# feihoo87/waveforms

Hardware: AMD Instinct MI355X
Metric: Msamples/s (all channels) (higher is better)
Workload: dtype f64; 1 GPU; sampler256: 256 ch/GPU x 1e+07 pts, 100 gaussian+DRAG pulses/ch, seeds 1000+c (SURVEY 8(d) C4/C5 channel spec), grid mode; channels_per_gpu=256, channels_total=256, points_per_channel=10000000, output=device (HBM) buffer, parallelism=channel-block-per-rank x1, no data-path collective

## Files before the change

### waveforms_amd/csrc/wfk_kernels.hip

```cpp
#include <hip/hip_runtime.h>

#include <string>
#include <type_traits>
#include <utility>

#include "wfk.h"
#include "wfk_internal.h"
#include "wfk_pick.h"

namespace {

__device__ __forceinline__ int uni(int v) { return __builtin_amdgcn_readfirstlane(v); }
__device__ __forceinline__ int64_t uni64(int64_t v) {
  const uint32_t lo = __builtin_amdgcn_readfirstlane((uint32_t)v);
  const uint32_t hi = __builtin_amdgcn_readfirstlane((uint32_t)((uint64_t)v >> 32));
  return (int64_t)(((uint64_t)hi << 32) | lo);
}
#define WFK_CONST __attribute__((address_space(4)))
template <typename V>
__device__ __forceinline__ V cload(const void* base, int byte_off) {
  return *reinterpret_cast<const WFK_CONST V*>(reinterpret_cast<uintptr_t>(base) + byte_off);
}
__device__ __forceinline__ DevPiece load_piece(const DevPiece* p) {
  DevPiece P;
// ... 392 lines not shown
      constexpr int IB = NS % 8 == 0 ? 8 : 1;
#pragma unroll
      for (int k0 = 0; k0 < NS; k0 += IB) {
        double dd[IB], f0[IB], s0[IB];
#pragma unroll
        for (int kk = 0; kk < IB; ++kk) {
          const double x = fma((double)(k0 + kk), D, u0);
          const double xc = fmin(fmax(x, start), stop);
          int j = (int)((xc - start) * inv_step);
          j = j > last ? last : j;
          const double d0 = xc - fma((double)j, step, start);
          dd[kk] = x != x ? x : d0;
          f0[kk] = fp[j];
          s0[kk] = sl[j];
        }
        __builtin_amdgcn_sched_barrier(0);
#pragma unroll
        for (int kk = 0; kk < IB; ++kk) prod[k0 + kk] *= (T)fma(s0[kk], dd[kk], f0[kk]);
      }
    } else if (mode == WFK_M_INTERP_GRID) {
#pragma clang fp contract(off)
      const double start = r[3], stop = r[4], inv_step = r[8], step = r[9];
      const int m = (int)r[5];
      const double* fp = a.pool + (int64_t)r[6];
      const double* sl = a.pool + (int64_t)r[7];
#pragma unroll
      for (int k0 = 0; k0 < NS; k0 += 4) {
        double xs[4], xj[4], f0[4], sv[4];
        int js[4];
        bool flat[4];
#pragma unroll
        for (int kk = 0; kk < 4; ++kk) {
          if (k0 + kk < NS) {
            double x = grid_time<SLICE>(a, j0 + 64 * (int64_t)(k0 + kk));
            if (tshift != 0.0) x = x - tshift;
            x = x - shift;
            int j;
            bool fl = true;
            if (!(x <= stop)) j = m - 1;
            else if (x < start) j = 0;
            else {
              j = (int)((x - start) * inv_step);
              j = j < 0 ? 0 : (j > m - 1 ? m - 1 : j);
              while (j > 0 && x < np_linspace_at_s(start, stop, m, j, step)) --j;
              while (j < m - 1 && x >= np_linspace_at_s(start, stop, m, j + 1, step)) ++j;
              fl = j == m - 1;
            }
            xs[kk] = x; js[kk] = j;
            xj[kk] = np_linspace_at_s(start, stop, m, j, step);
            flat[kk] = fl || xj[kk] == x;
          }
        }
#pragma unroll
        for (int kk = 0; kk < 4; ++kk)
          if (k0 + kk < NS) { f0[kk] = fp[js[kk]]; sv[kk] = sl[js[kk]]; }
#pragma unroll
        for (int kk = 0; kk < 4; ++kk) {
          if (k0 + kk < NS) {
            double v = flat[kk] ? f0[kk] : sv[kk] * (xs[kk] - xj[kk]) + f0[kk];
            if (isnan(xs[kk])) v = xs[kk];
            else if (isnan(v))
              v = prim_interp_fast(xs[kk], start, stop, fp, sl, m, inv_step, step);
            prod[k0 + kk] *= (T)v;
          }
        }
      }
    } else {
      const double D = r[3];
#pragma unroll
      for (int k = 0; k < NS; ++k) prod[k] *= (T)(u0 + (double)k * D);
    }
    return;
  }
  if (!DIRECT) return;
  const double pw = r[1];
  const bool has_pw = pw != 1.0;
  double* mine = s_val + threadIdx.x;
  if (mode == WFK_M_SAMPLED) {
    const double* tab = a.pool + (int64_t)r[3];
    const int64_t i0 = (int64_t)r[4], m = (int64_t)r[5];
#pragma unroll 1
    for (int k = 0; k < NS; ++k) {
      int64_t i = j0 + 64 * (int64_t)k - i0;
      i = i < 0 ? 0 : (i >= m ? m - 1 : i);
      double v = m > 0 ? tab[i] : __builtin_nan("");
      if (has_pw) v = np_power(v, pw);
      mine[k * WFK_WG] = v;
    }
  } else {
#pragma unroll 1
    for (int k = 0; k < NS; ++k) {
      double x = time_at<TLIST, SLICE>(a, j0 + 64 * (int64_t)k);
      if (tshift != 0.0) x = x - tshift;
      double v = prim_direct(mode, x - shift, r, a.pool);
      if (has_pw) v = np_power(v, pw);
      mine[k * WFK_WG] = v;
    }
  }
#pragma unroll
  for (int k = 0; k < NS; ++k) prod[k] *= (T)mine[k * WFK_WG];
}

struct FceSeeds { double c, s, g, r; };

__device__ __attribute__((noinline)) FceSeeds fce_seeds(double theta, double theta_lo, double ea,
                                                        double eb, int carrier, int env) {
#pragma clang fp contract(off)
  FceSeeds o;
  o.c = 1.0; o.s = 0.0; o.g = 1.0; o.r = 1.0;
  if (carrier == 1) {
    const double IPI_HI = 0.31830988618379069, IPI_LO = -1.9678676675182486e-17;
    const double xh = theta * IPI_HI;
    const double xl = fma(theta, IPI_HI, -xh) + fma(theta, IPI_LO, theta_lo * IPI_HI);
    const double n = rint(xh);
    double ss, cc;
    sincospi((xh - n) + xl, &ss, &cc);
    const bool odd = ((long long)n) & 1;
    o.s = odd ? -ss : ss;
    o.c = odd ? -cc : cc;
  }
  if (carrier == 2) o.c = erf(theta);
  if (env) {
    o.g = exp(ea);
    o.r = exp(eb);
  }
  return o;
}

struct CorrCtx {
  double dj0;
  double xref;
  double step, t0, tshift, last, dlast;
  int kbase;
};

template <int K>
__device__ __forceinline__ double corr_delta(const CorrCtx& cc, double dj0, double D, double W,
                                             double wm, double sm) {
#pragma clang fp contract(off)
  const double dj = dj0 + (double)(64 * K);
  const double m = dj * cc.step;
  double t = m + cc.t0;
  if (dj == cc.dlast) t = cc.last;
  t = t - cc.tshift;
  const double eps = (t - cc.xref) - (double)(cc.kbase + K) * D;
  const double um = t - sm;
  const double bb = um - t;
  const double eu = (t - (um - bb)) + (-sm - bb);
  const double pm = wm * um;
  const double rho = -__builtin_fma(wm, um, -pm);
  return __builtin_fma(W, eps, __builtin_fma(-wm, eu, rho));
}

template <typename T, int NS, int DEG, bool CARRIER, int ENV, bool CORR = false>
__device__ __forceinline__ void fce_loop(const double2* tab, const double* r, FceSeeds& sd,
                                         double u0, T (&acc)[NS],
                                         const CorrCtx* cc = nullptr) {
  using S = typename std::conditional<ENV == 2, double, T>::type;
  constexpr int SB = 4;
  asm volatile("" : "+v"(u0) : : "memory");
  double dj0 = 0.0, wm = 0.0, sm = 0.0;
  if constexpr (CORR) {
    wm = r[WFK_FCE_WM];
    sm = r[WFK_FCE_SM];
    dj0 = cc->dj0;
    asm volatile("" : "+v"(dj0));
  }
  const T c0 = (T)sd.c, s0 = (T)sd.s;
  const T A0 = (T)r[WFK_FCE_A], A1 = (T)r[WFK_FCE_A + 1], B0 = (T)r[WFK_FCE_B],
          B1 = (T)r[WFK_FCE_B + 1];
  const T A2 = DEG > 1 ? (T)r[WFK_FCE_A + 2] : (T)0, A3 = DEG > 1 ? (T)r[WFK_FCE_A + 3] : (T)0;
  const T B2 = DEG > 1 ? (T)r[WFK_FCE_B + 2] : (T)0, B3 = DEG > 1 ? (T)r[WFK_FCE_B + 3] : (T)0;
  const T ac = A0 * c0, as = A0 * s0;
  const bool fold = CARRIER && !CORR && DEG > 0;
  const T P0 = fold ? A0 * c0 + B0 * s0 : (T)0, P1 = fold ? A1 * c0 + B1 * s0 : (T)0;
  const T Q0 = fold ? B0 * c0 - A0 * s0 : (T)0, Q1 = fold ? B1 * c0 - A1 * s0 : (T)0;
  const T P2 = fold && DEG > 1 ? A2 * c0 + B2 * s0 : (T)0, P3 = fold && DEG > 1 ? A3 * c0 + B3 * s0 : (T)0;
  const T Q2 = fold && DEG > 1 ? B2 * c0 - A2 * s0 : (T)0, Q3 = fold && DEG > 1 ? B3 * c0 - A3 * s0 : (T)0;
  const double D = r[WFK_FCE_D];
  S g = (S)sd.g, rr = (S)sd.r;
  const S q = (S)r[WFK_FCE_Q];
  T u = (T)u0;
  const T Dt = (T)D;
  double2 tb[2][SB];
  if (CARRIER) {
    WFK_EACH(SB, kk) tb[0][kk] = tab[kk]; WFK_END
  }
  WFK_EACH(NS / SB, kb)
    if constexpr (CARRIER && (kb + 1) * SB < NS) {
      WFK_EACH(SB, kk) tb[(kb + 1) & 1][kk] = tab[(kb + 1) * SB + kk]; WFK_END
    }
    WFK_EACH(SB, kk)
      constexpr int k = kb * SB + kk;
      T val;
      if constexpr (DEG == 0 && CARRIER && !CORR && ENV == 0) {
        const double2 cs = tb[kb & 1][kk];
        acc[k] = __builtin_fma(ac, (T)cs.x, acc[k]);
        acc[k] = __builtin_fma(-as, (T)cs.y, acc[k]);
        return;
      }
      if (DEG == 0) {
        if (CARRIER) {
          const double2 cs = tb[kb & 1][kk];
          if constexpr (CORR) {
            const T we = (T)corr_delta<k>(*cc, dj0, D, r[WFK_FCE_W], wm, sm);
            const T ck = c0 * (T)cs.x - s0 * (T)cs.y;
            const T sk = s0 * (T)cs.x + c0 * (T)cs.y;
            val = A0 * (ck - we * sk);
          } else {
            val = ac * (T)cs.x - as * (T)cs.y;
          }
        } else {
          val = A0;
        }
      } else if constexpr (CARRIER && !CORR) {
        const double2 cs = tb[kb & 1][kk];
        T pp, qq;
        if (DEG == 1) {
          pp = P1 * u + P0;
          qq = Q1 * u + Q0;
        } else {
          pp = ((P3 * u + P2) * u + P1) * u + P0;
          qq = ((Q3 * u + Q2) * u + Q1) * u + Q0;
        }
        u += Dt;
        val = pp * (T)cs.x + qq * (T)cs.y;
      } else {
        T pa, pb;
        if (DEG == 1) {
          pa = A1 * u + A0;
          pb = B1 * u + B0;
        } else {
          pa = ((A3 * u + A2) * u + A1) * u + A0;
          pb = ((B3 * u + B2) * u + B1) * u + B0;
        }
        u += Dt;
        if (CARRIER) {
          const double2 cs = tb[kb & 1][kk];
          T ck = c0 * (T)cs.x - s0 * (T)cs.y;
          T sk = s0 * (T)cs.x + c0 * (T)cs.y;
          if constexpr (CORR) {
            const T we = (T)corr_delta<k>(*cc, dj0, D, r[WFK_FCE_W], wm, sm);
            const T c1 = ck - we * sk;
            sk = sk + we * ck;
            ck = c1;
          }
          val = pa * ck + pb * sk;
        } else {
          val = pa;
        }
      }
      if (ENV) {
        acc[k] += val * (T)g;
        g *= rr;
        rr *= q;
      } else {
        acc[k] += val;
      }
    WFK_END
    __builtin_amdgcn_sched_barrier(0);
  WFK_END
  if (ENV) {
    sd.g = (double)g;
    sd.r = (double)rr;
  }
  if (CARRIER) {
    const double2 e = tab[NS];
    const double c = sd.c, sn = sd.s;
    sd.c = c * e.x - sn * e.y;
    sd.s = sn * e.x + c * e.y;
  }
}

template <typename T, int NS, int DEG, bool CARRIER, bool CORR = false>
__device__ __forceinline__ void fce_env(const double2* tab, const double* r, FceSeeds& sd,
                                        double u0, int env, T (&acc)[NS], const CorrCtx* cc = nullptr) {
  if (env == 0) fce_loop<T, NS, DEG, CARRIER, 0, CORR>(tab, r, sd, u0, acc, cc);
  else if (sizeof(T) == 8 || env == 1) fce_loop<T, NS, DEG, CARRIER, 1, CORR>(tab, r, sd, u0, acc, cc);
  else fce_loop<T, NS, DEG, CARRIER, 2>(tab, r, sd, u0, acc);
}

template <bool EXACT = false>
__device__ __forceinline__ FceSeeds fce_make_seeds(const double* r, double x, int fl) {
  double v = (x - r[WFK_FCE_SG]) / r[WFK_FCE_SIGMA];
  const double Hh = r[WFK_FCE_H];
  if ((fl & 0x33) == 0x31) {
    const double vm = v + 0.5 * Hh;
    return fce_seeds(v, 0.0, -(vm * vm), -Hh * (2.0 * vm + Hh), 2, 1);
  }
  if (fl & WFK_FCE_EXPENV) v = 0.0;
  const double sref = r[WFK_FCE_SREF], W = r[WFK_FCE_W];
  const double d = x - sref;
  const double th = W * d;
  double lo = 0.0;
  if (EXACT) {
    const double bb = d - x;
    const double ed = (x - (d - bb)) + (-sref - bb);
    lo = fma(W, ed, fma(W, d, -th));
  }
  if (fl & WFK_FCE_EXPENV)
    return fce_seeds(th, lo, r[WFK_FCE_SIGMA] * (x - r[WFK_FCE_SG]), Hh, (fl >> 2) & 1, (fl >> 4) & 3);
  return fce_seeds(th, lo, -(v * v), -Hh * (2.0 * v + Hh), (fl >> 2) & 1, (fl >> 4) & 3);
}

template <typename T, int NS, bool CORR = false>
__device__ __forceinline__ void fce_eval(const double* blk, const double* r, FceSeeds& sd,
                                         double x, bool wide_env, T (&acc)[NS], int fl,
                                         const CorrCtx* cc = nullptr) {
  const int deg = fl & 3;
  const int carrier = (fl >> 2) & 1;
  int env = (fl >> 4) & 3;
  if (env && sizeof(T) == 4 && (wide_env || ((fl >> 6) & 1) == 0)) env = 2;
  const double2* tab = reinterpret_cast<const double2*>(blk + WFK_FCE_TABOFF(fl));
  const double u0 = x - r[WFK_FCE_SLIN];
  if constexpr (CORR && sizeof(T) == 8) {
    if (carrier && ((fl >> 7) & 1)) {
      if (deg == 0) fce_env<T, NS, 0, true, true>(tab, r, sd, u0, env, acc, cc);
      else if (deg == 1) fce_env<T, NS, 1, true, true>(tab, r, sd, u0, env, acc, cc);
      else fce_env<T, NS, 3, true, true>(tab, r, sd, u0, env, acc, cc);
      return;
    }
  }
  if (carrier) {
    if (deg == 0) fce_env<T, NS, 0, true>(tab, r, sd, u0, env, acc);
    else if (deg == 1) fce_env<T, NS, 1, true>(tab, r, sd, u0, env, acc);
    else fce_env<T, NS, 3, true>(tab, r, sd, u0, env, acc);
  } else {
    if (deg == 0) fce_env<T, NS, 0, false>(tab, r, sd, u0, env, acc);
    else fce_env<T, NS, 3, false>(tab, r, sd, u0, env, acc);
  }
}

template <typename T, int NS, bool CPLX>
__device__ __forceinline__ void fce_envmul(const double* r, FceSeeds& sd, T (&acc)[NS],
                                           T (&acci)[CPLX ? NS : 1]) {
  double g = sd.g, rr = sd.r;
  const double q = r[WFK_FCE_Q];
  WFK_EACH(NS, k)
    acc[k] *= (T)g;
    if constexpr (CPLX) acci[k] *= (T)g;
    g *= rr;
    rr *= q;
  WFK_END
  sd.g = g;
  sd.r = rr;
}

template <typename T, int NS, bool CPLX>
__device__ __forceinline__ void fce_erfmul(const double* r, FceSeeds& sd, double x, T (&acc)[NS],
                                           T (&acci)[CPLX ? NS : 1]) {
  double E = sd.c, g = sd.g, rr = sd.r;
  const double q = r[WFK_FCE_Q], h = r[WFK_FCE_H];
  const double m0 = r[WFK_FCE_A], m1 = r[WFK_FCE_A + 1];
  const double p0 = r[WFK_FCE_B], p1 = r[WFK_FCE_B + 1], p2 = r[WFK_FCE_B + 2], p3 = r[WFK_FCE_B + 3];
  double vm = (x - r[WFK_FCE_SG]) / r[WFK_FCE_SIGMA] + 0.5 * h;
  WFK_EACH(NS, k)
    const T m = (T)fma(m1, E, m0);
    acc[k] *= m;
    if constexpr (CPLX) acci[k] *= m;
    const double w = vm * vm;
    E = fma(g, fma(fma(fma(p3, w, p2), w, p1), w, p0), E);
    g *= rr;
    rr *= q;
    vm += h;
  WFK_END
  sd.c = E;
  sd.g = g;
  sd.r = rr;
}

template <typename T, int NS>
__device__ __forceinline__ void fce_bank(const double* blk, const double* gblk, const double* rec0, int n, double* s_st, int lane,
                                         T (&acc)[NS]) {
  constexpr int SB = 4;
#pragma unroll 1
  for (int i = 0; i < n; ++i) {
    const double* r = rec0 + i * WFK_FCE_REC;
    const int fl = uni(WFK_FCE_WORD(r));
#ifndef WFK_BANK_LDS
    const WFK_CONST double* tabd = reinterpret_cast<const WFK_CONST double*>(reinterpret_cast<uintptr_t>(gblk + WFK_FCE_TABOFF(fl)));
#else
    const double* tabd = blk + WFK_FCE_TABOFF(fl);
#endif
    auto tab = [&](int k) __attribute__((always_inline)) { return make_double2(tabd[2 * k], tabd[2 * k + 1]); };
    double* const st = s_st + WFK_FCE_STOFF(fl) + lane;
    const double c = st[0], sn = st[64];
    const double A0 = r[WFK_FCE_A];
    const T ac = (T)(A0 * c), as = (T)(A0 * sn);
    double2 tb[2][SB];
    WFK_EACH(SB, kk) tb[0][kk] = tab(kk); WFK_END
    WFK_EACH(NS / SB, kb)
      if constexpr ((kb + 1) * SB < NS) {
        WFK_EACH(SB, kk) tb[(kb + 1) & 1][kk] = tab((kb + 1) * SB + kk); WFK_END
      }
      WFK_EACH(SB, kk)
        constexpr int k = kb * SB + kk;
        const double2 cs = tb[kb & 1][kk];
        acc[k] = __builtin_fma(ac, (T)cs.x, acc[k]);
        acc[k] = __builtin_fma(-as, (T)cs.y, acc[k]);
      WFK_END
    WFK_END
    const double2 e = tab(NS);
    st[0] = c * e.x - sn * e.y;
    st[64] = sn * e.x + c * e.y;
  }
}

__device__ __forceinline__ double udbl(double v) {
  const uint64_t b = (uint64_t)__double_as_longlong(v);
  const uint32_t lo = __builtin_amdgcn_readfirstlane((uint32_t)b), hi = __builtin_amdgcn_readfirstlane((uint32_t)(b >> 32));
  return __longlong_as_double((long long)(((uint64_t)hi << 32) | lo));
}

template <typename T, int NS, bool CPLX>
__device__ __forceinline__ void fce_tabmul(const double* r, const KArgs& a, double x, T (&acc)[NS],
                                           T (&acci)[CPLX ? NS : 1]) {
  const double qmax = udbl(r[WFK_FCE_A + 1]), Dq = udbl(r[WFK_FCE_B]);
  double q = ((x - r[WFK_FCE_SLIN]) - r[WFK_FCE_A]) * r[WFK_FCE_A + 2];
  const double2* tab = uniptr(reinterpret_cast<const double2*>(a.pool) + uni64((int64_t)r[WFK_FCE_A + 3]));
  constexpr int IB = NS % 8 == 0 ? 8 : 1;
#pragma unroll
  for (int k0 = 0; k0 < NS; k0 += IB) {
    double fr[IB];
    double2 e[IB];
#pragma unroll
    for (int kk = 0; kk < IB; ++kk) {
      const double qc = fmin(fmax(q, 0.0), qmax);
      fr[kk] = __builtin_amdgcn_fract(qc);
      e[kk] = tab[(uint32_t)(int)qc];
      q += Dq;
    }
    __builtin_amdgcn_sched_barrier(0);
#pragma unroll
    for (int kk = 0; kk < IB; ++kk) {
      const T m = (T)fma(fr[kk], e[kk].y, e[kk].x);
      acc[k0 + kk] *= m;
      if constexpr (CPLX) acci[k0 + kk] *= m;
    }
  }
}

template <typename T, int NS, bool CPLX>
__device__ __forceinline__ void fce_mollmul(const double* r, double x, T (&acc)[NS], T (&acci)[CPLX ? NS : 1]) {
  const double u0 = x - r[WFK_FCE_SLIN];
  const double D = udbl(r[WFK_FCE_D]), ir = udbl(r[WFK_FCE_A]);
#pragma unroll
  for (int k = 0; k < NS; ++k) {
    const double xx = fma((double)k, D, u0) * ir;
    const double q = fma(xx, xx, -1.0);
    const double qq = q < -1e-300 ? q : -1.0;
    const double v = exp_inline(rcp_nr(qq) + 1.0);
    const T m = (T)(q < 0.0 ? v : 0.0);
    acc[k] *= m;
    if constexpr (CPLX) acci[k] *= m;
    if ((k & 3) == 3) __builtin_amdgcn_sched_barrier(0);
  }
}

template <typename T, int NS>
__device__ __forceinline__ void fce_ownmul(const double* blk, const double* r, const KArgs& a, double x, double* st,
                                           int fl, T (&acc)[NS]) {
  const bool car = (fl & 4) != 0;
  double c = 1.0, sn = 0.0;
  if (car) { c = st[0]; sn = st[64]; }
  const double A0 = r[WFK_FCE_A];
  const double ac = A0 * c, as = A0 * sn;
  const double2* ptab = reinterpret_cast<const double2*>(blk + WFK_FCE_TABOFF(fl));
  if (uni((int)r[WFK_FCE_B + 3]) == 0) {
    const double qmax = udbl(r[WFK_FCE_A + 1]), Dq = udbl(r[WFK_FCE_B + 1]);
    double q = ((x - r[WFK_FCE_SLIN]) - r[WFK_FCE_B + 2]) * r[WFK_FCE_A + 2];
    const double2* tab = uniptr(reinterpret_cast<const double2*>(a.pool) + uni64((int64_t)r[WFK_FCE_A + 3]));
    constexpr int IB = NS % 8 == 0 ? 8 : 1;
#pragma unroll
    for (int k0 = 0; k0 < NS; k0 += IB) {
      double fr[IB];
      double2 e[IB];
#pragma unroll
      for (int kk = 0; kk < IB; ++kk) {
        const double qc = fmin(fmax(q, 0.0), qmax);
        fr[kk] = __builtin_amdgcn_fract(qc);
        e[kk] = tab[(uint32_t)(int)qc];
        q += Dq;
// ... 99 lines not shown


__device__ __forceinline__ void sincos_small(double th, double& c, double& s) {
  const double n = rint(th * 0.63661977236758138);
  double r = fma(-n, 1.57079632679489655800e+00, th);
  r = fma(-n, 6.12323399573676603587e-17, r);
  const double z = r * r;
  double ps = fma(z, 1.58969099521155010221e-10, -2.50507602534068634195e-08);
  ps = fma(z, ps, 2.75573137070700676789e-06);
  ps = fma(z, ps, -1.98412698298579493134e-04);
  ps = fma(z, ps, 8.33333333332248946124e-03);
  ps = fma(z, ps, -1.66666666666666324348e-01);
  const double sr = fma(z * r, ps, r);
  double pc = fma(z, -1.13596475577881948265e-11, 2.08757232129817482790e-09);
  pc = fma(z, pc, -2.75573143513906633035e-07);
  pc = fma(z, pc, 2.48015872894767294178e-05);
  pc = fma(z, pc, -1.38888888888741095749e-03);
  pc = fma(z, pc, 4.16666666666666019037e-02);
  const double cr = fma(z * z, pc, fma(z, -0.5, 1.0));
  const int q = (int)n;
  const double a = (q & 1) ? sr : cr, b = (q & 1) ? cr : sr;
  c = ((q + 1) & 2) ? -a : a;
  s = (q & 2) ? -b : b;
}

template <typename T, int NS, bool CPLX, bool CUBIC, bool CARRIER, int ENV>
__device__ __forceinline__ void fce_point_shape(const double* r, const double (&x)[NS], T (&acc)[NS],
                                                T (&acci)[CPLX ? NS : 1], bool imag) {
  auto ud = [](double v) __attribute__((always_inline)) {
    return __hiloint2double(uni(__double2hiint(v)), uni(__double2loint(v)));
  };
  const double A0 = ud(r[WFK_FCE_A]), A1 = ud(r[WFK_FCE_A + 1]), B0 = ud(r[WFK_FCE_B]), B1 = ud(r[WFK_FCE_B + 1]);
  const double A2 = CUBIC ? ud(r[WFK_FCE_A + 2]) : 0.0, A3 = CUBIC ? ud(r[WFK_FCE_A + 3]) : 0.0;
  const double B2 = CUBIC ? ud(r[WFK_FCE_B + 2]) : 0.0, B3 = CUBIC ? ud(r[WFK_FCE_B + 3]) : 0.0;
  const double W = ud(r[WFK_FCE_W]), sref = ud(r[WFK_FCE_SREF]), slin = ud(r[WFK_FCE_SLIN]);
  const double sg = ud(r[WFK_FCE_SG]), ea = ud(ENV == 1 ? r[WFK_FCE_H] : r[WFK_FCE_SIGMA]);
  constexpr int PB = NS % 4 == 0 ? 4 : 1;
#pragma unroll
  for (int k0 = 0; k0 < NS; k0 += PB) {
  double val[PB];
#pragma unroll
  for (int kk = 0; kk < PB; ++kk) {
    const int k = k0 + kk;
    const double u = x[k] - slin;
    double A, Bq;
    if constexpr (CUBIC) {
      A = fma(fma(fma(A3, u, A2), u, A1), u, A0);
      Bq = fma(fma(fma(B3, u, B2), u, B1), u, B0);
    } else {
      A = fma(A1, u, A0);
      Bq = fma(B1, u, B0);
    }
    double v = A;
    if constexpr (CARRIER) {
      double c, sn;
      sincos_small(W * (x[k] - sref), c, sn);
      v = fma(Bq, sn, A * c);
    }
    if constexpr (ENV != 0) {
      double q = (x[k] - sg) * ea;
      if constexpr (ENV == 1) q = -(q * q);
      v *= exp_inline(q);
    }
    val[kk] = v;
  }
#pragma unroll
  for (int kk = 0; kk < PB; ++kk) {
    const int k = k0 + kk;
    if constexpr (CPLX) {
      if (imag) acci[k] += (T)val[kk];
      else acc[k] += (T)val[kk];
    } else {
      acc[k] += (T)val[kk];
    }
  }
  __builtin_amdgcn_sched_barrier(0);
  }
}

template <typename T, int NS, bool CPLX>
__device__ __forceinline__ void fce_point(const double* r, const double (&x)[NS], T (&acc)[NS],
                                          T (&acci)[CPLX ? NS : 1]) {
  const int fl = uni(WFK_FCE_WORD(r));
  const int deg = fl & 3, env = (fl >> 4) & 3;
  const bool carrier = (fl & 4) != 0, imag = (fl & 8) != 0;
  if (imag && !CPLX) return;
  if (env == 3) {
    const double sg = r[WFK_FCE_SG], isig = r[WFK_FCE_H];
#pragma unroll
    for (int k = 0; k < NS; ++k) {
      const double v = (x[k] - sg) * isig;
      const T e = (T)exp_inline(-(v * v));
      acc[k] *= e;
      if constexpr (CPLX) acci[k] *= e;
    }
    return;
  }
  const int ev = env == 0 ? 0 : ((fl & WFK_FCE_EXPENV) ? 2 : 1);
  if (carrier && !(fl & WFK_FCE_TLSMALL)) {
    const double W = r[WFK_FCE_W], sref = r[WFK_FCE_SREF], slin = r[WFK_FCE_SLIN], sg = r[WFK_FCE_SG];
    const double ea = ev == 1 ? r[WFK_FCE_H] : r[WFK_FCE_SIGMA];
#pragma unroll 1
    for (int k = 0; k < NS; ++k) {
      const double u = x[k] - slin;
      double A = r[WFK_FCE_A + 3], Bq = r[WFK_FCE_B + 3];
      for (int i = 2; i >= 0; --i) { A = fma(A, u, r[WFK_FCE_A + i]); Bq = fma(Bq, u, r[WFK_FCE_B + i]); }
      const double2 cs = sincos_phase(W * (x[k] - sref));
      double v = fma(Bq, cs.y, A * cs.x);
      if (ev) { double q = (x[k] - sg) * ea; if (ev == 1) q = -(q * q); v *= exp_inline(q); }
      static_for<NS>([&](auto kk) __attribute__((always_inline)) {
        if (decltype(kk)::value == k) {
          if constexpr (CPLX) { if (imag) acci[decltype(kk)::value] += (T)v; else acc[decltype(kk)::value] += (T)v; }
          else acc[decltype(kk)::value] += (T)v;
        }
      });
    }
    return;
  }
  const bool cubic = deg > 1;
#define WFK_PT(CU, CA, EN) fce_point_shape<T, NS, CPLX, CU, CA, EN>(r, x, acc, acci, imag)
  if (!cubic) {
    if (carrier) { if (ev == 1) WFK_PT(false, true, 1); else if (ev == 2) WFK_PT(false, true, 2); else WFK_PT(false, true, 0); }
    else { if (ev == 1) WFK_PT(false, false, 1); else if (ev == 2) WFK_PT(false, false, 2); else WFK_PT(false, false, 0); }
  } else {
    if (carrier) { if (ev == 1) WFK_PT(true, true, 1); else if (ev == 2) WFK_PT(true, true, 2); else WFK_PT(true, true, 0); }
    else { if (ev == 1) WFK_PT(true, false, 1); else if (ev == 2) WFK_PT(true, false, 2); else WFK_PT(true, false, 0); }
  }
#undef WFK_PT
}

template <typename T> struct OutOps;
template <> struct OutOps<double> {
  using Real = double;
  using Cplx = double2;
};
template <> struct OutOps<float> {
  using Real = float;
  using Cplx = float2;
};

template <typename T>
__device__ __forceinline__ T clip_np(T v, T lo, T hi) {
  v = v < lo ? lo : v;
  v = v > hi ? hi : v;
  return v;
}

template <typename T>
__device__ __forceinline__ void clip_np_cplx(T& re, T& im, T lo, T hi) {
  if (re < lo || (re == lo && im < (T)0)) { re = lo; im = (T)0; }
  if (re > hi || (re == hi && im > (T)0)) { re = hi; im = (T)0; }
}

template <typename T, bool CPLX, int NS, bool PLAIN, bool NT = false, typename E = T>
__device__ __forceinline__ void store_tile_impl(const KArgs& a, const DevChannel& C,
                                                const DevPiece& P, typename OutOps<E>::Real* tr,
                                                typename OutOps<E>::Cplx* tc, int64_t w0, int lane,
                                                const T (&acc)[NS],
                                                const T (&acci)[CPLX ? NS : 1]) {
  using OutC = typename OutOps<E>::Cplx;
  constexpr int WT = 64 * NS;
  const T base = (T)C.offset;
  const bool clip = !PLAIN && C.do_clip && (P.flags & WFK_PF_HAS_TERMS);
  const bool accum = !PLAIN && a.accumulate != 0;
  const T lo = (T)C.clip_lo, hi = (T)C.clip_hi;
  const int lo_l = (int)(P.start - w0 > 0 ? P.start - w0 : 0);
  const int hi_l = (int)(P.stop - w0 < WT ? P.stop - w0 : WT);
  WFK_EACH(NS, k)
    const int o = lane + 64 * k;
    if (PLAIN || (o >= lo_l && o < hi_l)) {
      T v = acc[k];
      T vi = (T)0;
      if constexpr (CPLX) vi = acci[k];
      if (clip) {
        if constexpr (CPLX) clip_np_cplx(v, vi, lo, hi);
        else v = clip_np(v, lo, hi);
      }
      v += base;
      if constexpr (CPLX) {
        if (accum) {
          const OutC old = tc[o];
          v += (T)old.x;
          vi += (T)old.y;
        }
        OutC w;
        w.x = (E)v;
        w.y = (E)vi;
        if constexpr (NT) {
          __builtin_nontemporal_store(w.x, &tc[o].x);
          __builtin_nontemporal_store(w.y, &tc[o].y);
        } else {
          tc[o] = w;
        }
      } else {
        if (accum) v += (T)tr[o];
        if constexpr (NT) __builtin_nontemporal_store((E)v, &tr[o]);
        else tr[o] = (E)v;
      }
    }
  WFK_END
}

template <typename T, bool CPLX, int NS, bool NT = false, typename E = T>
__device__ __forceinline__ void store_tile(const KArgs& a, const DevChannel& C, const DevPiece& P,
                                           typename OutOps<E>::Real* tr,
                                           typename OutOps<E>::Cplx* tc, int64_t w0, int lane,
                                           const T (&acc)[NS], const T (&acci)[CPLX ? NS : 1]) {
  const bool full = P.start <= w0 && P.stop >= w0 + 64 * NS;
  const bool clip = C.do_clip && (P.flags & WFK_PF_HAS_TERMS);
  if (full && !clip && !a.accumulate)
    store_tile_impl<T, CPLX, NS, true, NT, E>(a, C, P, tr, tc, w0, lane, acc, acci);
  else
    store_tile_impl<T, CPLX, NS, false, NT, E>(a, C, P, tr, tc, w0, lane, acc, acci);
}

__device__ __forceinline__ int64_t xcd_chunk(const KArgs& a) {
  const int64_t b = blockIdx.x;
  const int64_t per = (a.n_chunks + 7) >> 3;
  const int64_t c = (b & 7) * per + (b >> 3);
  return c < a.n_chunks ? a.chunk_base + c : -1;
}

template <typename T, bool CPLX, int NS, bool CORR, int FAM>
#ifndef WFK_LEAN_WAVES
#define WFK_LEAN_WAVES 3
#endif
#ifndef WFK_LEAN_WAVES_F32
#define WFK_LEAN_WAVES_F32 4
#endif
__global__ void __launch_bounds__(64, (sizeof(T) == 4 ? WFK_LEAN_WAVES_F32 : WFK_LEAN_WAVES) - (CPLX ? 1 : 0) -
                                          (CORR && sizeof(T) == 8 && !CPLX ? 1 : 0))
wfk_sample_lean(const KArgs a) {
  extern __shared__ __attribute__((aligned(16))) double s_dyn[];
  double* const s_par = s_dyn;
  double* const s_st = s_dyn + a.lean_par;
  constexpr int WT = 64 * NS;
  using OutR = typename OutOps<T>::Real;
  using OutC = typename OutOps<T>::Cplx;

  const int lane = threadIdx.x;
  const int64_t chunk = xcd_chunk(a);
  if (chunk < 0) return;
  const int ch = uni((int)(chunk / a.chunks_per_ch));
  const int64_t cc = uni64(chunk - (int64_t)ch * a.chunks_per_ch);
  const DevChannel C = a.channels[ch];
  int p = uni(a.chunk_first[chunk]);
  DevPiece cur = load_piece(a.pieces + p);
  int64_t staged = -1;
  int state_piece = -1;
  int64_t state_w0 = -1;
  int since_seed = 0;
  int cs_age = 0;

  OutR* const outr = uniptr(reinterpret_cast<OutR*>(a.out) + (int64_t)ch * a.ch_stride);
  OutC* const outc = uniptr(reinterpret_cast<OutC*>(a.out) + (int64_t)ch * a.ch_stride);

  for (int tt = 0; tt < a.tiles_per_chunk; ++tt) {
    const int64_t w0 = uni64((cc * a.tiles_per_chunk + tt) * WT);
    if (w0 >= a.n) break;
    const int64_t w1 = w0 + WT < a.n ? w0 + WT : a.n;
    const int64_t j0 = w0 + lane;
    while (p < C.piece_end - 1 && cur.stop <= w0) {
      p = uni(p + 1);
      cur = load_piece(a.pieces + p);
    }

    for (int q = p;;) {
      const DevPiece P = cur;
      if (P.start >= w1) break;
      T acc[NS], acci[CPLX ? NS : 1];
      WFK_EACH(NS, k) acc[k] = (T)0; WFK_END
      WFK_EACH(CPLX ? NS : 1, k) acci[k] = (T)0; WFK_END
      const bool mine = !a.mixed || P.n_blk == 0 || (P.flags & WFK_PF_LEAN);
      if (P.n_blk != 0 && mine) {
        if (P.par_off != staged) {
          __syncthreads();
          for (int i = lane; i < P.first_len; i += 64) s_par[i] = a.params[P.par_off + i];
          __syncthreads();
          staged = P.par_off;
        }
        const int nops = uni((int)s_par[1]);
        double x = grid_time(a, j0);
        if (C.tshift != 0.0) x = x - C.tshift;
        const bool valid = state_piece == q && state_w0 == w0;
        const bool carried = valid && since_seed < a.reseed;
        if (!carried) {
          bool seed_cs = true;
          if constexpr (!CORR) {
            seed_cs = !valid || cs_age >= WFK_LEAN_RESEED_CS;
          }
          if (seed_cs) cs_age = 0;
          for (int op = 0; op < nops; ++op) {
            const double* srec = s_par + WFK_BLK_HDR + op * WFK_FCE_REC;
            const int sfl = uni(WFK_FCE_WORD(srec));
            if constexpr (!CORR) {
              if (!seed_cs && (sfl & (WFK_FCE_HAS_CS | WFK_FCE_HAS_GR | WFK_FCE_CHIRP)) == WFK_FCE_HAS_CS) continue;
            }
            if constexpr (FAM >= 2) {
              if (sfl & WFK_FCE_CHIRP) {
                const ChirpSeeds cd = chirp_make_seeds(srec, x, sfl);
                double* ct = s_st + WFK_FCE_STOFF(sfl) + lane;
                ct[0] = cd.c; ct[64] = cd.s; ct[128] = cd.wc; ct[192] = cd.ws;
                if (sfl & WFK_FCE_HAS_GR) { ct[256] = cd.g; ct[320] = cd.r; }
                continue;
              }
            }
            if constexpr (FAM >= 3) {
              if ((sfl & 0x32) == 0x32) continue;
            }
            const FceSeeds sd = fce_make_seeds<CORR>(srec, x, sfl);
            double* st = s_st + WFK_FCE_STOFF(sfl) + lane;
            if (sfl & WFK_FCE_HAS_CS) {
              st[0] = sd.c;
              st[64] = sd.s;
              st += 128;
            }
            if (sfl & WFK_FCE_HAS_GR) {
              st[0] = sd.g;
              st[64] = sd.r;
            }
          }
          since_seed = 0;
        }
        CorrCtx cc;
        if constexpr (CORR) {
          const int64_t js = j0 - (int64_t)since_seed * WT;
          double xs = grid_time(a, js);
          if (C.tshift != 0.0) xs = xs - C.tshift;
          cc.dj0 = (double)(j0 + a.i0);
          cc.xref = xs;
          cc.step = a.step; cc.t0 = a.t0; cc.tshift = C.tshift; cc.last = a.last;
          cc.dlast = a.has_last ? (double)(a.i0 + a.n - 1) : -1.0;
          cc.kbase = since_seed * NS;
        }
        for (int op = 0; op < nops; ++op) {
          FceSeeds sd;
          const double* rec = s_par + WFK_BLK_HDR + op * WFK_FCE_REC;
          const int fl = uni(WFK_FCE_WORD(rec));
          double* const st = s_st + WFK_FCE_STOFF(fl) + lane;
          if constexpr (FAM >= 2) {
            if (fl & WFK_FCE_CHIRP) {
              ChirpSeeds cd;
              cd.c = st[0]; cd.s = st[64]; cd.wc = st[128]; cd.ws = st[192];
              cd.g = 1.0; cd.r = 1.0;
              const bool cenv = (fl & WFK_FCE_HAS_GR) != 0;
              if (cenv) { cd.g = st[256]; cd.r = st[320]; }
              const double cu0 = x - rec[WFK_FCE_SLIN];
              if (fl & 8) {
                if constexpr (CPLX) {
                  if (cenv) chirp_loop<T, NS, true>(rec, cd, cu0, acci); else chirp_loop<T, NS, false>(rec, cd, cu0, acci);
                }
              } else {
                if (cenv) chirp_loop<T, NS, true>(rec, cd, cu0, acc); else chirp_loop<T, NS, false>(rec, cd, cu0, acc);
              }
              st[0] = cd.c; st[64] = cd.s; st[128] = cd.wc; st[192] = cd.ws;
              if (cenv) { st[256] = cd.g; st[320] = cd.r; }
              continue;
            }
          }
          if constexpr (FAM >= 1) {
            if (fl & WFK_FCE_BANK) {
              const int nb = uni((int)rec[WFK_FCE_SIGMA]);
              if (fl & 8) {
                if constexpr (CPLX) fce_bank<T, NS>(s_par, a.params + P.par_off, rec, nb, s_st, lane, acci);
              } else {
                fce_bank<T, NS>(s_par, a.params + P.par_off, rec, nb, s_st, lane, acc);
              }
              op += nb - 1;
              continue;
            }
          }
          if constexpr (FAM >= 4) {
            if (fl < 0) {
              if (fl & 8) {
                if constexpr (CPLX) fce_ownmul<T, NS>(s_par, rec, a, x, st, fl, acci);
              } else {
                fce_ownmul<T, NS>(s_par, rec, a, x, st, fl, acc);
              }
              continue;
            }
          }
          if constexpr (FAM >= 3) {
            if ((fl & 0x32) == 0x32) {
              if (fl & 1) fce_mollmul<T, NS, CPLX>(rec, x, acc, acci);
              else fce_tabmul<T, NS, CPLX>(rec, a, x, acc, acci);
              continue;
            }
          }
          double* const stg = st + ((fl & (WFK_FCE_HAS_CS | WFK_FCE_HAS_GR)) == (WFK_FCE_HAS_CS | WFK_FCE_HAS_GR) ? 128 : 0);
          sd.c = st[0];
          sd.s = st[64];
          sd.g = stg[0];
          sd.r = stg[64];
          if (FAM >= 1 && ((fl >> 4) & 3) == 3) {
            if constexpr (FAM >= 1) {
              if (fl & 3) fce_erfmul<T, NS, CPLX>(rec, sd, x, acc, acci);
              else fce_envmul<T, NS, CPLX>(rec, sd, acc, acci);
            }
          } else if (fl & 8) {
            if constexpr (CPLX) fce_eval<T, NS, CORR>(s_par, rec, sd, x, true, acci, fl, &cc);
          } else {
            fce_eval<T, NS, CORR>(s_par, rec, sd, x, true, acc, fl, &cc);
          }
          if (fl & WFK_FCE_HAS_CS) {
            st[0] = sd.c;
            st[64] = sd.s;
          }
          if (fl & WFK_FCE_HAS_GR) {
            stg[0] = sd.g;
            stg[64] = sd.r;
          }
        }
        state_piece = q;
        state_w0 = w0 + WT;
        ++since_seed;
        ++cs_age;
      }
      if (mine) store_tile<T, CPLX, NS, CORR>(a, C, P, uniptr(outr + w0), uniptr(outc + w0), w0, lane, acc, acci);
      if (P.stop >= w1 || q + 1 >= C.piece_end) break;
      q = uni(q + 1);
      cur = load_piece(a.pieces + q);
      p = q;
    }
  }
}

#ifndef WFK_TL_WGS
#define WFK_TL_WGS 3
#endif
template <typename T, bool CPLX, bool TLIST, bool GENERIC, bool DIRECT, int NS>
__global__ void __launch_bounds__(WFK_WG, TLIST ? WFK_TL_WGS : ((DIRECT || GENERIC) ? 2 : 1)) wfk_sample(const KArgs a);
template <typename T, typename E, bool CPLX, bool TLIST, bool GENERIC, bool DIRECT, int NS, bool SLICE>
__device__ __forceinline__ void wfk_sample_body(const KArgs& a) {
  __shared__ __attribute__((aligned(16))) double s_par_all[WFK_LDS_DOUBLES];
  __shared__ double s_val[DIRECT ? NS * WFK_WG : 1];
  constexpr int WT = 64 * NS;
  constexpr int TILE = WFK_WG * NS;
  using OutR = typename OutOps<E>::Real;
  using OutC = typename OutOps<E>::Cplx;

  const int lane = threadIdx.x & 63;
  const int wave = uni(threadIdx.x >> 6);
  constexpr bool WP = TLIST && NS == 1;
  const bool wp = WP && a.wavepriv != 0;
  double* const s_par = (WP && wp) ? s_par_all + wave * (WFK_LDS_DOUBLES / 4) : s_par_all;
  const int64_t chunk = xcd_chunk(a);
  if (chunk < 0) return;
  const int ch = uni((int)(chunk / a.chunks_per_ch));
  const int64_t cc = uni64(chunk - (int64_t)ch * a.chunks_per_ch);
  const DevChannel C = a.channels[ch];
  int p = uni(a.chunk_first[chunk]);
  int64_t staged = -1;

  OutR* const outr = uniptr(reinterpret_cast<OutR*>(a.out) + (int64_t)ch * a.ch_stride);
  OutC* const outc = uniptr(reinterpret_cast<OutC*>(a.out) + (int64_t)ch * a.ch_stride);

  for (int tt = 0; tt < a.tiles_per_chunk; ++tt) {
    const int64_t g0 = uni64((cc * a.tiles_per_chunk + tt) * TILE);
    if (g0 >= a.n) break;
    const int64_t g1 = g0 + TILE < a.n ? g0 + TILE : a.n;
    const int64_t w0 = uni64(g0 + (int64_t)wave * WT);
    const int64_t j0 = w0 + lane;
    while (p < C.piece_end - 1 && cload<int64_t>(a.pieces + p, offsetof(DevPiece, stop)) <= g0)
      p = uni(p + 1);

    for (int q = p; q < C.piece_end; q = uni(q + 1)) {
      const DevPiece P = load_piece(a.pieces + q);
      if (P.start >= g1) break;
      if constexpr (TLIST && !GENERIC && !DIRECT) {
        if (a.mixed && P.n_blk != 0 && !(P.flags & WFK_PF_LEAN)) continue;
      } else {
        if (a.mixed && (P.n_blk == 0 || (P.flags & (WFK_PF_LEAN | WFK_PF_SHORT)))) continue;
      }
      const bool active = w0 < a.n && P.start < w0 + WT && P.stop > w0;

      T acc[NS], acci[CPLX ? NS : 1];
#pragma unroll
      for (int k = 0; k < NS; ++k) acc[k] = (T)0;
      if (CPLX) {
#pragma unroll
        for (int k = 0; k < NS; ++k) acci[k] = (T)0;
      }

      double tx[(TLIST && !GENERIC && !DIRECT) ? NS : 1];
      if constexpr (TLIST && !GENERIC && !DIRECT) {
        if (active) {
#pragma unroll
          for (int i = 0; i < NS; ++i) {
            tx[i] = time_at<true>(a, j0 + 64 * (int64_t)i);
            if (C.tshift != 0.0) tx[i] = tx[i] - C.tshift;
          }
        }
      }

      int64_t off = P.par_off;
      int len = P.first_len;
      for (int b = 0; b < P.n_blk; ++b) {
        if (WP && wp) {
          if (active && off != staged) {
            for (int i = lane; i < len; i += 64) s_par[i] = a.params[off + i];
            staged = off;
          }
        } else if (off != staged) {
          __syncthreads();
          for (int i = threadIdx.x; i < len; i += WFK_WG) s_par[i] = a.params[off + i];
          __syncthreads();
          staged = off;
        }
        if (active) {
          const int nops = uni((int)s_par[1]);
          int pos = WFK_BLK_HDR;
          for (int k = 0; k < nops; ++k) {
            const int kind = uni((int)s_par[pos]);
            if constexpr (TLIST && !GENERIC && !DIRECT) {
              if (kind == WFK_OP_FCE) {
                fce_point<T, NS, CPLX>(s_par + pos, tx, acc, acci);
                pos += WFK_FCE_REC;
                continue;
              }
            }
            if (!TLIST && kind == WFK_OP_FCE) {
              const int fl = uni(WFK_FCE_WORD(s_par + pos));
              if (((fl >> 4) & 3) == 3) {
                double x = grid_time<SLICE>(a, j0);
                if (C.tshift != 0.0) x = x - C.tshift;
                FceSeeds sd = fce_make_seeds(s_par + pos, x, fl);
                if (fl & 3) fce_erfmul<T, NS, CPLX>(s_par + pos, sd, x, acc, acci);
                else fce_envmul<T, NS, CPLX>(s_par + pos, sd, acc, acci);
              } else if (fl & 8) {
                if constexpr (CPLX) apply_fce<T, NS, SLICE>(s_par, s_par + pos, a, C.tshift, j0, acci);
              } else {
                apply_fce<T, NS, SLICE>(s_par, s_par + pos, a, C.tshift, j0, acc);
              }
              pos += WFK_FCE_REC;
              continue;
            }
            if (!GENERIC) continue;
            const T ar = (T)s_par[pos + 1], ai = (T)s_par[pos + 2];
            const int nf = uni((int)s_par[pos + 3]);
            pos += WFK_TERM_HDR;
            T prod[NS];
#pragma unroll
            for (int i = 0; i < NS; ++i) prod[i] = (T)1;
            for (int f = 0; f < nf; ++f) {
              apply_factor<T, TLIST, DIRECT, NS, SLICE>(s_par, s_par + pos, a, C.tshift, j0, prod, s_val);
              pos += WFK_FREC;
            }
#pragma unroll
            for (int i = 0; i < NS; ++i) acc[i] += ar * prod[i];
            if (CPLX) {
#pragma unroll
              for (int i = 0; i < NS; ++i) acci[i] += ai * prod[i];
            }
          }
        }
        off += len;
        if (b + 1 < P.n_blk) len = (int)a.params[off];
      }

      if (active)
        store_tile<T, CPLX, NS, false, E>(a, C, P, uniptr(outr + w0), uniptr(outc + w0), w0, lane, acc, acci);
    }
  }
}

template <typename T, bool CPLX, bool TLIST, bool GENERIC, bool DIRECT, int NS>
__global__ void __launch_bounds__(WFK_WG, TLIST ? WFK_TL_WGS : ((DIRECT || GENERIC) ? 2 : 1)) wfk_sample(const KArgs a) {
  wfk_sample_body<T, T, CPLX, TLIST, GENERIC, DIRECT, NS, false>(a);
}
#ifndef WFK_SLICE_CPLX_WGS
#define WFK_SLICE_CPLX_WGS 1
// ... 77 lines not shown
```

Before: 744,800 Msamples/s.

## Trim per-tile overhead: init accumulators from first op, incremental time, skip zero offset

The first pulse operation now writes the accumulators directly instead of adding into zeroed registers. Tile time is computed incrementally from a running double index rather than through grid_time on every tile. The time computation is hoisted out of the piece loop. A store variant skips adding the channel offset when it is exactly zero, and accumulation is made explicitly unfused with asm barriers to keep results bitwise identical. This removes some FLOPs and zeroing per tile, but adds template variants and code size, and may constrain scheduling.

```diff
diff --git a/waveforms_amd/csrc/wfk_kernels.hip b/waveforms_amd/csrc/wfk_kernels.hip
--- a/waveforms_amd/csrc/wfk_kernels.hip
+++ b/waveforms_amd/csrc/wfk_kernels.hip
@@ -568,7 +568,24 @@
   return __builtin_fma(W, eps, __builtin_fma(-wm, eu, rho));
 }
 
-template <typename T, int NS, int DEG, bool CARRIER, int ENV, bool CORR = false>
+enum { WFK_ACC_SUNK = 0, WFK_ACC_ADD = 1, WFK_ACC_INIT = 2 };
+
+template <typename T>
+__device__ __forceinline__ T fce_mul_rounded(T a, T b) {
+#pragma clang fp contract(off)
+  return a * b;
+}
+
+template <int ACC, typename T>
+__device__ __forceinline__ void fce_put(T& acc, T v) {
+#pragma clang fp contract(off)
+  static_assert(ACC != WFK_ACC_SUNK, "flavour 0 is written out in the loop");
+  if constexpr (ACC == WFK_ACC_INIT) acc = v;
+  else acc = acc + v;
+  asm("" : "+v"(acc));
+}
+
+template <typename T, int NS, int DEG, bool CARRIER, int ENV, bool CORR = false, int ACC = WFK_ACC_SUNK>
 __device__ __forceinline__ void fce_loop(const double2* tab, const double* r, FceSeeds& sd,
                                          double u0, T (&acc)[NS],
                                          const CorrCtx* cc = nullptr) {
@@ -611,8 +628,13 @@
       T val;
       if constexpr (DEG == 0 && CARRIER && !CORR && ENV == 0) {
         const double2 cs = tb[kb & 1][kk];
-        acc[k] = __builtin_fma(ac, (T)cs.x, acc[k]);
+        if constexpr (ACC == WFK_ACC_INIT) {
+          acc[k] = fce_mul_rounded(ac, (T)cs.x);
+        } else {
+          acc[k] = __builtin_fma(ac, (T)cs.x, acc[k]);
+        }
         acc[k] = __builtin_fma(-as, (T)cs.y, acc[k]);
+        if constexpr (ACC != WFK_ACC_SUNK) asm("" : "+v"(acc[k]));
         return;
       }
       if (DEG == 0) {
@@ -667,11 +689,13 @@
         }
       }
       if (ENV) {
-        acc[k] += val * (T)g;
+        if constexpr (ACC == WFK_ACC_SUNK) acc[k] += val * (T)g;
+        else fce_put<ACC>(acc[k], fce_mul_rounded(val, (T)g));
         g *= rr;
         rr *= q;
       } else {
-        acc[k] += val;
+        if constexpr (ACC == WFK_ACC_SUNK) acc[k] += val;
+        else fce_put<ACC>(acc[k], val);
       }
     WFK_END
     __builtin_amdgcn_sched_barrier(0);
@@ -688,12 +712,12 @@
   }
 }
 
-template <typename T, int NS, int DEG, bool CARRIER, bool CORR = false>
+template <typename T, int NS, int DEG, bool CARRIER, bool CORR = false, int ACC = WFK_ACC_SUNK>
 __device__ __forceinline__ void fce_env(const double2* tab, const double* r, FceSeeds& sd,
                                         double u0, int env, T (&acc)[NS], const CorrCtx* cc = nullptr) {
-  if (env == 0) fce_loop<T, NS, DEG, CARRIER, 0, CORR>(tab, r, sd, u0, acc, cc);
-  else if (sizeof(T) == 8 || env == 1) fce_loop<T, NS, DEG, CARRIER, 1, CORR>(tab, r, sd, u0, acc, cc);
-  else fce_loop<T, NS, DEG, CARRIER, 2>(tab, r, sd, u0, acc);
+  if (env == 0) fce_loop<T, NS, DEG, CARRIER, 0, CORR, ACC>(tab, r, sd, u0, acc, cc);
+  else if (sizeof(T) == 8 || env == 1) fce_loop<T, NS, DEG, CARRIER, 1, CORR, ACC>(tab, r, sd, u0, acc, cc);
+  else fce_loop<T, NS, DEG, CARRIER, 2, false, ACC>(tab, r, sd, u0, acc);
 }
 
 template <bool EXACT = false>
@@ -719,7 +743,7 @@
   return fce_seeds(th, lo, -(v * v), -Hh * (2.0 * v + Hh), (fl >> 2) & 1, (fl >> 4) & 3);
 }
 
-template <typename T, int NS, bool CORR = false>
+template <typename T, int NS, bool CORR = false, int ACC = WFK_ACC_SUNK>
 __device__ __forceinline__ void fce_eval(const double* blk, const double* r, FceSeeds& sd,
                                          double x, bool wide_env, T (&acc)[NS], int fl,
                                          const CorrCtx* cc = nullptr) {
@@ -731,19 +755,19 @@
   const double u0 = x - r[WFK_FCE_SLIN];
   if constexpr (CORR && sizeof(T) == 8) {
     if (carrier && ((fl >> 7) & 1)) {
-      if (deg == 0) fce_env<T, NS, 0, true, true>(tab, r, sd, u0, env, acc, cc);
-      else if (deg == 1) fce_env<T, NS, 1, true, true>(tab, r, sd, u0, env, acc, cc);
-      else fce_env<T, NS, 3, true, true>(tab, r, sd, u0, env, acc, cc);
+      if (deg == 0) fce_env<T, NS, 0, true, true, ACC>(tab, r, sd, u0, env, acc, cc);
+      else if (deg == 1) fce_env<T, NS, 1, true, true, ACC>(tab, r, sd, u0, env, acc, cc);
+      else fce_env<T, NS, 3, true, true, ACC>(tab, r, sd, u0, env, acc, cc);
       return;
     }
   }
   if (carrier) {
-    if (deg == 0) fce_env<T, NS, 0, true>(tab, r, sd, u0, env, acc);
-    else if (deg == 1) fce_env<T, NS, 1, true>(tab, r, sd, u0, env, acc);
-    else fce_env<T, NS, 3, true>(tab, r, sd, u0, env, acc);
+    if (deg == 0) fce_env<T, NS, 0, true, false, ACC>(tab, r, sd, u0, env, acc);
+    else if (deg == 1) fce_env<T, NS, 1, true, false, ACC>(tab, r, sd, u0, env, acc);
+    else fce_env<T, NS, 3, true, false, ACC>(tab, r, sd, u0, env, acc);
   } else {
-    if (deg == 0) fce_env<T, NS, 0, false>(tab, r, sd, u0, env, acc);
-    else fce_env<T, NS, 3, false>(tab, r, sd, u0, env, acc);
+    if (deg == 0) fce_env<T, NS, 0, false, false, ACC>(tab, r, sd, u0, env, acc);
+    else fce_env<T, NS, 3, false, false, ACC>(tab, r, sd, u0, env, acc);
   }
 }
 
@@ -1149,7 +1173,7 @@
   if (re > hi || (re == hi && im > (T)0)) { re = hi; im = (T)0; }
 }
 
-template <typename T, bool CPLX, int NS, bool PLAIN, bool NT = false, typename E = T>
+template <typename T, bool CPLX, int NS, bool PLAIN, bool NT = false, typename E = T, bool BARE = false>
 __device__ __forceinline__ void store_tile_impl(const KArgs& a, const DevChannel& C,
                                                 const DevPiece& P, typename OutOps<E>::Real* tr,
                                                 typename OutOps<E>::Cplx* tc, int64_t w0, int lane,
@@ -1173,7 +1197,7 @@
         if constexpr (CPLX) clip_np_cplx(v, vi, lo, hi);
         else v = clip_np(v, lo, hi);
       }
-      v += base;
+      if constexpr (!BARE) v += base;
       if constexpr (CPLX) {
         if (accum) {
           const OutC old = tc[o];
@@ -1198,14 +1222,16 @@
   WFK_END
 }
 
-template <typename T, bool CPLX, int NS, bool NT = false, typename E = T>
+template <typename T, bool CPLX, int NS, bool NT = false, typename E = T, bool ZB = false>
 __device__ __forceinline__ void store_tile(const KArgs& a, const DevChannel& C, const DevPiece& P,
                                            typename OutOps<E>::Real* tr,
                                            typename OutOps<E>::Cplx* tc, int64_t w0, int lane,
                                            const T (&acc)[NS], const T (&acci)[CPLX ? NS : 1]) {
   const bool full = P.start <= w0 && P.stop >= w0 + 64 * NS;
   const bool clip = C.do_clip && (P.flags & WFK_PF_HAS_TERMS);
-  if (full && !clip && !a.accumulate)
+  if (ZB && full && !clip && !a.accumulate && ((uint64_t)__double_as_longlong(C.offset) << 1) == 0)
+    store_tile_impl<T, CPLX, NS, true, NT, E, true>(a, C, P, tr, tc, w0, lane, acc, acci);
+  else if (full && !clip && !a.accumulate)
     store_tile_impl<T, CPLX, NS, true, NT, E>(a, C, P, tr, tc, w0, lane, acc, acci);
   else
     store_tile_impl<T, CPLX, NS, false, NT, E>(a, C, P, tr, tc, w0, lane, acc, acci);
@@ -1216,6 +1242,23 @@
   const int64_t per = (a.n_chunks + 7) >> 3;
   const int64_t c = (b & 7) * per + (b >> 3);
   return c < a.n_chunks ? a.chunk_base + c : -1;
+}
+
+__device__ __forceinline__ double lean_time(double dj, double step, double t0) {
+#pragma clang fp contract(off)
+  const double m = dj * step;
+  return m + t0;
+}
+
+template <int FAM>
+__device__ __forceinline__ bool lean_first_inits(int fl) {
+  if (fl & 8) return false;
+  if (FAM >= 2 && (fl & WFK_FCE_CHIRP)) return false;
+  if (FAM >= 1 && (fl & WFK_FCE_BANK)) return false;
+  if (FAM >= 4 && fl < 0) return false;
+  if (FAM >= 3 && (fl & 0x32) == 0x32) return false;
+  if (FAM >= 1 && ((fl >> 4) & 3) == 3) return false;
+  return true;
 }
 
 template <typename T, bool CPLX, int NS, bool CORR, int FAM>
@@ -1234,6 +1277,8 @@
   constexpr int WT = 64 * NS;
   using OutR = typename OutOps<T>::Real;
   using OutC = typename OutOps<T>::Cplx;
+  constexpr bool TRIM = !(sizeof(T) == 4 && !CPLX && FAM == 4) && !(CORR && CPLX && FAM == 1);
+  constexpr int ADD = TRIM ? WFK_ACC_ADD : WFK_ACC_SUNK;
 
   const int lane = threadIdx.x;
   const int64_t chunk = xcd_chunk(a);
@@ -1252,7 +1297,10 @@
   OutR* const outr = uniptr(reinterpret_cast<OutR*>(a.out) + (int64_t)ch * a.ch_stride);
   OutC* const outc = uniptr(reinterpret_cast<OutC*>(a.out) + (int64_t)ch * a.ch_stride);
 
-  for (int tt = 0; tt < a.tiles_per_chunk; ++tt) {
+  double dj = TRIM ? (double)(cc * a.tiles_per_chunk * WT + lane + a.i0) : 0.0;
+  const double tsh = C.tshift != 0.0 ? C.tshift : 0.0;
+
+  for (int tt = 0; tt < a.tiles_per_chunk; ++tt, dj += (double)WT) {
     const int64_t w0 = uni64((cc * a.tiles_per_chunk + tt) * WT);
     if (w0 >= a.n) break;
     const int64_t w1 = w0 + WT < a.n ? w0 + WT : a.n;
@@ -1261,12 +1309,24 @@
       p = uni(p + 1);
       cur = load_piece(a.pieces + p);
     }
+    double x;
+    if constexpr (TRIM) {
+      x = lean_time(dj, a.step, a.t0);
+      if (a.has_last && w1 == a.n) {
+        asm volatile("");
+        if (j0 == a.n - 1) x = a.last;
+      }
+      x = x - tsh;
+    } else {
+      x = grid_time(a, j0);
+      if (C.tshift != 0.0) x = x - C.tshift;
+    }
 
     for (int q = p;;) {
       const DevPiece P = cur;
       if (P.start >= w1) break;
       T acc[NS], acci[CPLX ? NS : 1];
-      WFK_EACH(NS, k) acc[k] = (T)0; WFK_END
+      const auto zero_acc = [&]() __attribute__((always_inline)) { WFK_EACH(NS, k) acc[k] = (T)0; WFK_END };
       WFK_EACH(CPLX ? NS : 1, k) acci[k] = (T)0; WFK_END
       const bool mine = !a.mixed || P.n_blk == 0 || (P.flags & WFK_PF_LEAN);
       if (P.n_blk != 0 && mine) {
@@ -1277,8 +1337,6 @@
           staged = P.par_off;
         }
         const int nops = uni((int)s_par[1]);
-        double x = grid_time(a, j0);
-        if (C.tshift != 0.0) x = x - C.tshift;
         const bool valid = state_piece == q && state_w0 == w0;
         const bool carried = valid && since_seed < a.reseed;
         if (!carried) {
@@ -1321,15 +1379,22 @@
         }
         CorrCtx cc;
         if constexpr (CORR) {
-          const int64_t js = j0 - (int64_t)since_seed * WT;
-          double xs = grid_time(a, js);
-          if (C.tshift != 0.0) xs = xs - C.tshift;
-          cc.dj0 = (double)(j0 + a.i0);
-          cc.xref = xs;
+          if constexpr (TRIM) {
+            const double xs = lean_time(dj - (double)(since_seed * WT), a.step, a.t0) - tsh;
+            cc.dj0 = dj;
+            cc.xref = since_seed == 0 ? x : xs;
+          } else {
+            double xs = grid_time(a, j0 - (int64_t)since_seed * WT);
+            if (C.tshift != 0.0) xs = xs - C.tshift;
+            cc.dj0 = (double)(j0 + a.i0);
+            cc.xref = xs;
+          }
           cc.step = a.step; cc.t0 = a.t0; cc.tshift = C.tshift; cc.last = a.last;
           cc.dlast = a.has_last ? (double)(a.i0 + a.n - 1) : -1.0;
           cc.kbase = since_seed * NS;
         }
+        const bool init = TRIM && nops > 0 && lean_first_inits<FAM>(uni(WFK_FCE_WORD(s_par + WFK_BLK_HDR)));
+        if (!init) zero_acc();
         for (int op = 0; op < nops; ++op) {
           FceSeeds sd;
           const double* rec = s_par + WFK_BLK_HDR + op * WFK_FCE_REC;
@@ -1395,9 +1460,11 @@
               else fce_envmul<T, NS, CPLX>(rec, sd, acc, acci);
             }
           } else if (fl & 8) {
-            if constexpr (CPLX) fce_eval<T, NS, CORR>(s_par, rec, sd, x, true, acci, fl, &cc);
+            if constexpr (CPLX) fce_eval<T, NS, CORR, ADD>(s_par, rec, sd, x, true, acci, fl, &cc);
+          } else if (TRIM && init && op == 0) {
+            if constexpr (TRIM) fce_eval<T, NS, CORR, WFK_ACC_INIT>(s_par, rec, sd, x, true, acc, fl, &cc);
           } else {
-            fce_eval<T, NS, CORR>(s_par, rec, sd, x, true, acc, fl, &cc);
+            fce_eval<T, NS, CORR, ADD>(s_par, rec, sd, x, true, acc, fl, &cc);
           }
           if (fl & WFK_FCE_HAS_CS) {
             st[0] = sd.c;
@@ -1412,8 +1479,10 @@
         state_w0 = w0 + WT;
         ++since_seed;
         ++cs_age;
-      }
-      if (mine) store_tile<T, CPLX, NS, CORR>(a, C, P, uniptr(outr + w0), uniptr(outc + w0), w0, lane, acc, acci);
+      } else {
+        zero_acc();
+      }
+      if (mine) store_tile<T, CPLX, NS, CORR, T, TRIM>(a, C, P, uniptr(outr + w0), uniptr(outc + w0), w0, lane, acc, acci);
       if (P.stop >= w1 || q + 1 >= C.piece_end) break;
       q = uni(q + 1);
       cur = load_piece(a.pieces + q);
```

Result: slower. 737,400 Msamples/s (-1.0%).
